# barathanaslan/whisper-ipa

Hardware: AMD Instinct MI355X
Metric: audio-seconds/sec transcribed (whisper-small, 30s clips) (higher is better)
Workload: dtype bf16

## Files before the change

### include/wipa.h

```cpp
#ifndef WIPA_H
#define WIPA_H
#include <stddef.h>
#include <stdint.h>
#ifdef __cplusplus
extern "C" {
#endif

typedef void* wipa_stream_t;

enum { WIPA_F32 = 0, WIPA_BF16 = 1, WIPA_FP8_E4M3 = 2  };
enum { WIPA_OK = 0, WIPA_ERR_ARG = -1, WIPA_ERR_HIP = -2, WIPA_ERR_STATE = -3 };

#define WIPA_N_SAMPLES 480000
#define WIPA_N_FRAMES 3000
#define WIPA_N_FFT 400
#define WIPA_HOP 160
#define WIPA_HEAD_DIM 64

int wipa_version(void);
const char* wipa_last_error(void);

int wipa_stream_create(wipa_stream_t* out);
int wipa_stream_create_cu_limited(int n_cus, wipa_stream_t* out);
int wipa_stream_destroy(wipa_stream_t s);
// ... 122 lines not shown
    const float* slabs;
    const float* bias_o;
    const float* ln_w;
    const float* ln_b;
    const void* wq;
    const float* bq;
    const void* kv;
    void* out;
    int64_t slab_stride;
    int32_t n_slabs, B, d, H, Tk, dtype;
    float eps, qk_scale;
    int32_t cross_splits;
} wipa_cross_block_desc;
int wipa_decode_cross_block(const wipa_cross_block_desc* d, wipa_stream_t s);

int wipa_cross_absorbed_splits(int want, int Tk);
int wipa_cross_absorbed_resident_groups_for(int B, int d, int Tk, int n_splits, int64_t budget_bytes);
int wipa_cross_absorbed_resident_groups(int B, int d, int Tk, int n_splits);
size_t wipa_cross_absorbed_scratch_bytes(int B, int d, int Tk);
int wipa_cross_absorbed_init(int d);
int wipa_cross_absorbed_attention(const void* q, int64_t q_row_stride, const void* wkT, const void* xa, const void* wv, const float* bv,
                                  void* out, int64_t out_row_stride, void* scratch, size_t scratch_bytes, int B, int H, int d, int Tk,
                                  float k_scale, int n_splits, wipa_stream_t s);
int wipa_decode_cross_absorbed_block(const wipa_cross_block_desc* c, const void* wkT, const void* wv, const float* bv, void* scratch,
                                     size_t scratch_bytes, wipa_stream_t s);
int wipa_decode_cross_absorbed_block_out(const wipa_cross_block_desc* c, const void* wkT, const void* wv, const float* bv, const void* wo,
                                         const float* bo, float* slabs_out, int64_t slab_stride, void* scratch, size_t scratch_bytes,
                                         wipa_stream_t s);
int wipa_cross_absorbed_stream(const void* xa, void* scratch, size_t scratch_bytes, int B, int H, int d, int Tk, int n_splits,
                               wipa_stream_t s);

int wipa_greedy_step(const float* logits, int64_t ldl, int B, int V, const float* mask_first,
                     const float* mask_always, int32_t* tokens, int64_t ld_tok, const int32_t* pos_dev, int n_init,
                     int eot, float* sum_logprobs, int32_t* not_done, wipa_stream_t s);
int wipa_add_i32(int32_t* p, int32_t v, wipa_stream_t s);
int wipa_greedy_step_embed(const float* logits, int64_t ldl, int B, int V, const float* mask_first, const float* mask_always,
                           int32_t* tokens, int64_t ld_tok, int32_t* pos_dev, int64_t* posd_dev, int32_t* done_counter, int n_init,
                           int eot, float* sum_logprobs, int32_t* not_done, const void* tok_emb, int emb_dtype,
                           const float* emb_scale, const float* pos_emb, int n_ctx, float* x, const float* ln_w, const float* ln_b,
                           void* y, int y_dtype, int D, float eps, wipa_stream_t s);
#define WIPA_GREEDY_PARTS 2048
int wipa_logits_greedy_supported(int B, int V, int d, int dtype);
size_t wipa_logits_greedy_partials_bytes(int B);
int wipa_logits_greedy(const void* x, int64_t ldx, const void* w, int64_t ldw, float* logits, int64_t ldl, int B, int V, int d,
                       const float* mask_first, const float* mask_always, const int32_t* pos_dev, int n_init, float* partials,
                       size_t partials_bytes, wipa_stream_t s);
// ... 105 lines not shown
```

### whisper_ipa_amd/_lib.py

```python
from __future__ import annotations

import ctypes as C
import os
import threading

_HERE = os.path.dirname(os.path.abspath(__file__))
LIB_PATH = os.path.join(_HERE, "libwipa.so")

WIPA_F32, WIPA_BF16, WIPA_FP8_E4M3 = 0, 1, 2
GREEDY_PARTS = 2048
ENC_GLOBAL, ENC_PER_LAYER = 7, 14
DEC_GLOBAL, DEC_PER_LAYER, DEC_FP8_PER_LAYER = 4, 20, 6
GEMM_DISPATCH = ("tile128", "tile256", "tile384", "tile384n", "tile256p", "skinny", "skinny_fp8", "skinny_ln", "kmajor", "split_k",
                 "tile_fp8", "tile_fp8_384")
ENC_FP8_PER_LAYER = 8
DEC_ABSORBED_PER_LAYER = 1

c_void_p, c_int, c_int64, c_size_t, c_float = C.c_void_p, C.c_int, C.c_int64, C.c_size_t, C.c_float


class GemmDesc(C.Structure):
    _fields_ = [
        ("A", c_void_p), ("W", c_void_p), ("C", c_void_p), ("bias", c_void_p), ("residual", c_void_p),
        ("pos", c_void_p), ("c_offset_dev", c_void_p),
# ... 76 lines not shown
                               c_float, c_void_p]),
    "wipa_layernorm_fp8": (c_int, [c_void_p, c_int64, c_void_p, c_int64, c_void_p, c_void_p, c_void_p, c_int, c_int, c_float, c_void_p]),
    "wipa_rowquant_fp8": (c_int, [c_void_p, c_int, c_int64, c_void_p, c_int64, c_void_p, c_int, c_int, c_void_p]),
    "wipa_add_slabs_layernorm": (c_int, [c_void_p, c_int64, c_void_p, c_int, c_int64, c_void_p, c_int, c_int64, c_void_p,
                                         c_void_p, c_int, c_int, c_float, c_void_p]),
    "wipa_embed_tokens": (c_int, [c_void_p, c_int64, c_int, c_int, c_int, c_void_p, c_void_p, c_int, c_void_p, c_void_p, c_void_p,
                                  c_int, c_void_p]),
    "wipa_attention": (c_int, [_P(AttnDesc), c_void_p]),
    "wipa_flash_attn_enc_f32": (c_int, [c_void_p, c_int64, c_void_p, c_int64, c_void_p, c_int64, c_void_p, c_int64, c_int, c_int,
                                       c_int, c_int, c_void_p]),
    "wipa_flash_attn_enc_bf16": (c_int, [c_void_p, c_int64, c_void_p, c_int64, c_void_p, c_int64, c_int, c_int, c_int,
                                         c_void_p]),
    "wipa_decode_attn": (c_int, [_P(AttnDesc), c_void_p]),
    "wipa_decode_cross_attn": (c_int, [c_void_p, c_void_p, c_void_p, c_int, c_int, c_int, c_int, c_void_p]),
    "wipa_decode_self_block": (c_int, [_P(SelfBlockDesc), c_void_p]),
    "wipa_decode_cross_block": (c_int, [_P(CrossBlockDesc), c_void_p]),
    "wipa_cross_absorbed_splits": (c_int, [c_int, c_int]),
    "wipa_cross_absorbed_resident_groups_for": (c_int, [c_int, c_int, c_int, c_int, c_int64]),
    "wipa_cross_absorbed_resident_groups": (c_int, [c_int, c_int, c_int, c_int]),
    "wipa_cross_absorbed_scratch_bytes": (c_size_t, [c_int, c_int, c_int]),
    "wipa_cross_absorbed_init": (c_int, [c_int]),
    "wipa_cross_absorbed_attention": (c_int, [c_void_p, c_int64, c_void_p, c_void_p, c_void_p, c_void_p, c_void_p, c_int64, c_void_p, c_size_t,
                                              c_int, c_int, c_int, c_int, c_float, c_int, c_void_p]),
    "wipa_cross_absorbed_stream": (c_int, [c_void_p, c_void_p, c_size_t, c_int, c_int, c_int, c_int, c_int, c_void_p]),
    "wipa_decode_cross_absorbed_block": (c_int, [_P(CrossBlockDesc), c_void_p, c_void_p, c_void_p, c_void_p, c_size_t, c_void_p]),
    "wipa_decode_cross_absorbed_block_out": (c_int, [_P(CrossBlockDesc), c_void_p, c_void_p, c_void_p, c_void_p, c_void_p, c_void_p, c_int64,
                                                     c_void_p, c_size_t, c_void_p]),
    "wipa_greedy_step": (c_int, [c_void_p, c_int64, c_int, c_int, c_void_p, c_void_p, c_void_p, c_int64, c_void_p, c_int,
                                 c_int, c_void_p, c_void_p, c_void_p]),
    "wipa_add_i32": (c_int, [c_void_p, C.c_int32, c_void_p]),
    "wipa_greedy_step_embed": (c_int, [c_void_p, c_int64, c_int, c_int, c_void_p, c_void_p, c_void_p, c_int64, c_void_p, c_void_p, c_void_p,
                                       c_int, c_int, c_void_p, c_void_p, c_void_p, c_int, c_void_p, c_void_p, c_int, c_void_p, c_void_p,
                                       c_void_p, c_void_p, c_int, c_int, c_float, c_void_p]),
    "wipa_logits_greedy_supported": (c_int, [c_int, c_int, c_int, c_int]),
    "wipa_logits_greedy_partials_bytes": (c_size_t, [c_int]),
    "wipa_logits_greedy": (c_int, [c_void_p, c_int64, c_void_p, c_int64, c_void_p, c_int64, c_int, c_int, c_int, c_void_p, c_void_p, c_void_p,
                                   c_int, c_void_p, c_size_t, c_void_p]),
    "wipa_greedy_step_embed_partials": (c_int, [c_void_p, c_int, c_int, c_void_p, c_int64, c_void_p, c_void_p, c_void_p, c_int, c_int, c_void_p,
                                                c_void_p, c_void_p, c_int, c_void_p, c_void_p, c_int, c_void_p, c_void_p, c_void_p, c_void_p,
                                                c_int, c_int, c_float, c_void_p]),
    "wipa_embed_layernorm": (c_int, [c_void_p, c_int64, c_int, c_void_p, c_void_p, c_int, c_void_p, c_void_p, c_int, c_void_p, c_void_p,
                                     c_void_p, c_void_p, c_int, c_int, c_float, c_void_p]),
    "wipa_bpe_create": (c_void_p, [c_void_p, c_void_p, c_void_p, c_int]),
    "wipa_bpe_free": (None, [c_void_p]),
    "wipa_bpe_encode_piece": (c_int, [c_void_p, C.c_char_p, c_int, c_void_p, c_int]),
    "wipa_bpe_decode": (c_int, [c_void_p, c_void_p, c_int, c_void_p, c_int]),
# ... 68 lines not shown
```

### whisper_ipa_amd/csrc/cross_absorbed.hip

```cpp
#include <cstdlib>
#include <mutex>
#include <type_traits>

#include "attn_stream.h"
#include "wipa_common.h"

namespace {

constexpr int FT = 32;
constexpr long long XA_RESIDENT_MB_SHARED = 16;
constexpr long long XA_RESIDENT_MB_LONE = -1;
typedef __attribute__((address_space(3))) void* lds_ptr_a;
typedef int v2i32 __attribute__((ext_vector_type(2)));

struct AbsParams {
    const __bf16* qp;
    const __bf16* xa;
    float* part_m;
    float* part_l;
    float* part_o;
    int Tk, n_splits, tiles_per_split, H;
    int resident_groups;
};

constexpr int POLICY_DEFAULT = 0, POLICY_NT = 2;

__device__ __forceinline__ int swz(int row) { return (row & 7) << 1; }

template <int D>
struct AbsCfg {
    static constexpr int NW = 4;
    static constexpr int ROWB = D * 2;
    static constexpr int TILE = FT * ROWB;
    static constexpr int SX = NW * 2 * 64 * 4 * (int)sizeof(float);
    static constexpr int NBUF = (3 * TILE + SX <= 160 * 1024) ? 3 : 2;
    static constexpr int SMEM = NBUF * TILE + SX;
};

template <int D>
__global__ __launch_bounds__(512, 1) void cross_absorbed_kernel(AbsParams p) {
    typedef AbsCfg<D> X;
    constexpr int NW = X::NW, ROWB = X::ROWB, TILE = X::TILE, NBUF = X::NBUF;
    constexpr int NDMA = TILE / 1024 / NW;
    constexpr int KS = D / NW / 32;
    constexpr int CT = D / NW / 16;
    static_assert(D % (32 * NW) == 0 && TILE % (1024 * NW) == 0, "width");
    extern __shared__ __attribute__((aligned(1024))) char smem[];
    float* sx = reinterpret_cast<float*>(smem + NBUF * TILE);
    const int tid = threadIdx.x, lane = tid & 63;
    const int wave = __builtin_amdgcn_readfirstlane(tid >> 6);
    const int l15 = lane & 15, g = lane >> 4;
    const int split = blockIdx.x, b = blockIdx.y;
    const int tile0 = split * p.tiles_per_split;
    const int n_tiles_total = (p.Tk + FT - 1) / FT;
    const int nt = max(0, min(p.tiles_per_split, n_tiles_total - tile0));
    const __bf16* xb = p.xa + (int64_t)b * p.Tk * D;

    bf16x8 qf[KS];
    {
        const __bf16* qr = p.qp + ((int64_t)b * 16 + l15) * D + wave * (D / NW) + 8 * g;
#pragma unroll
        for (int ks = 0; ks < KS; ++ks) qf[ks] = *reinterpret_cast<const bf16x8*>(qr + 32 * ks);
    }
    const __amdgpu_buffer_rsrc_t rX = __builtin_amdgcn_make_buffer_rsrc((void*)xb, 0, 0x7fffffff, 0x00020000);
    int drow[NDMA], dch[NDMA];
#pragma unroll
    for (int i = 0; i < NDMA; ++i) {
        const int off = 1024 * (NDMA * wave + i) + 16 * lane;
        drow[i] = off / ROWB;
        dch[i] = ((off % ROWB) >> 4) ^ swz(off / ROWB);
    }
    const int res_tiles = p.resident_groups / 2;
    auto stage_as = [&](auto policy, int t, int buf) {
        constexpr int AUX = decltype(policy)::value;
        const int f0 = (tile0 + t) * FT;
#pragma unroll
        for (int i = 0; i < NDMA; ++i) {
            const int voff = min(f0 + drow[i], p.Tk - 1) * ROWB + dch[i] * 16;
            __builtin_amdgcn_raw_ptr_buffer_load_lds(rX, (lds_ptr_a)(smem + buf * TILE + 1024 * (NDMA * wave + i)), 16, voff, 0, 0, AUX);
// ... 156 lines not shown
typedef __bf16 bf16x4v __attribute__((ext_vector_type(4)));

template <int D, int NW_>
struct AbsCfg2 {
    static constexpr int NWV = NW_;
    static constexpr int GF = 16;
    static constexpr int ROWB = D * 2;
    static constexpr int SLOT = GF * ROWB;
    static constexpr int SMEM_LOOP = NWV * 2 * SLOT;
    static constexpr int MROW = D + 4;
    static constexpr int SMEM_MERGE = NWV * 16 * MROW * 4 + NWV * 32 * 4;
    static constexpr int SMEM = SMEM_LOOP > SMEM_MERGE ? SMEM_LOOP : SMEM_MERGE;
};

#define WIPA_TR8(X, A, IMM)                                                                                                          \
    asm volatile("ds_read_b64_tr_b16 %0, %8 offset:" #IMM "\n\tds_read_b64_tr_b16 %1, %9 offset:" #IMM                              \
                 "\n\tds_read_b64_tr_b16 %2, %10 offset:" #IMM "\n\tds_read_b64_tr_b16 %3, %11 offset:" #IMM                          \
                 "\n\tds_read_b64_tr_b16 %4, %12 offset:" #IMM "\n\tds_read_b64_tr_b16 %5, %13 offset:" #IMM                          \
                 "\n\tds_read_b64_tr_b16 %6, %14 offset:" #IMM "\n\tds_read_b64_tr_b16 %7, %15 offset:" #IMM "\n\ts_waitcnt lgkmcnt(0)" \
                 : "=&v"(X[0]), "=&v"(X[1]), "=&v"(X[2]), "=&v"(X[3]), "=&v"(X[4]), "=&v"(X[5]), "=&v"(X[6]), "=&v"(X[7])           \
                 : "v"(A[0]), "v"(A[1]), "v"(A[2]), "v"(A[3]), "v"(A[4]), "v"(A[5]), "v"(A[6]), "v"(A[7])                           \
                 : "memory")

template <int D, int NW_>
__global__ __launch_bounds__(64 * NW_, 1) void cross_absorbed_v2_kernel(AbsParams p) {
    typedef AbsCfg2<D, NW_> X;
    constexpr int NWV = X::NWV, GF = X::GF, ROWB = X::ROWB, SLOT = X::SLOT;
    constexpr int NDMA = SLOT / 1024;
    constexpr int KS = D / 32;
    constexpr int CT = D / 16;
    static_assert(SLOT % 1024 == 0 && NDMA <= 32 && CT % 8 == 0 && KS % 4 == 0 && CT / 8 <= 8 && D % 128 == 0, "width");
    extern __shared__ __attribute__((aligned(1024))) char smem[];
    const int tid = threadIdx.x, lane = tid & 63;
    const int wave = __builtin_amdgcn_readfirstlane(tid >> 6);
    const int l15 = lane & 15, g = lane >> 4;
    const int split = blockIdx.x, b = blockIdx.y;
    const int groups_total = (p.Tk + GF - 1) / GF;
    const int gps = 2 * p.tiles_per_split;
    const int g0 = split * gps;
    const int ng = max(0, min(gps, groups_total - g0));
    const int my_n = ng > wave ? (ng - wave + NWV - 1) / NWV : 0;
    const __bf16* xb = p.xa + (int64_t)b * p.Tk * D;
    char* my = smem + wave * (2 * SLOT);

    bf16x8 qf[KS];
    {
        const __bf16* qr = p.qp + ((int64_t)b * 16 + l15) * D + 8 * g;
#pragma unroll
        for (int ks = 0; ks < KS; ++ks) qf[ks] = *reinterpret_cast<const bf16x8*>(qr + 32 * ks);
    }
    const __amdgpu_buffer_rsrc_t rX = __builtin_amdgcn_make_buffer_rsrc((void*)xb, 0, 0x7fffffff, 0x00020000);
    constexpr int G1K = (ROWB % 1024 == 0) ? 1024 : ((ROWB % 512 == 0) ? 512 : 256);
    constexpr int PER = ROWB / G1K, QR = 1024 / G1K;
    static_assert(NDMA % PER == 0 && PER <= 3 && (QR == 1 || QR == 2 || QR == 4), "transfer / row period");
    int dma_a[PER], dma_b[PER];
#pragma unroll
    for (int t = 0; t < PER; ++t) {
        const int off = 1024 * t + 16 * lane;
        const int r = off / ROWB, c = (off - r * ROWB) >> 4;
        dma_a[t] = (c ^ (r << 1)) << 4;
        dma_b[t] = r * ROWB;
    }
    int lane_v = lane;
    auto stage_as = [&](auto policy, int i_local, int slot) {
        constexpr int AUX = decltype(policy)::value;
// ... 492 lines not shown
        for (int e = tid; e < (16 - CG) * 64; e += 512) qh[CG + (e >> 6)][e & 63] = (__bf16)0.f;
    }
    __syncthreads();
    {
        const bf16x8 a0 = *reinterpret_cast<const bf16x8*>(&qh[l15][8 * g]);
        const bf16x8 a1 = *reinterpret_cast<const bf16x8*>(&qh[l15][32 + 8 * g]);
#pragma unroll
        for (int i = 0; i < NTW; ++i) {
            const int nt = wave * NTW + i;
            if (nt < NT) {
                f32x4 acc = {0.f, 0.f, 0.f, 0.f};
                acc = __builtin_amdgcn_mfma_f32_16x16x32_bf16(a0, wkf[i][0], acc, 0, 0, 0);
                acc = __builtin_amdgcn_mfma_f32_16x16x32_bf16(a1, wkf[i][1], acc, 0, 0, 0);
#pragma unroll
                for (int r = 0; r < 4; ++r) {
                    const int bb_ = b0 + 4 * g + r;
                    if (4 * g + r < CG && bb_ < p.B) p.qp[((int64_t)bb_ * 16 + h) * D + 16 * nt + l15] = (__bf16)(acc[r] * p.k_scale);
                }
            }
        }
    }
}

template <int D>
int launch_attn(const AbsParams& p_in, int B, hipStream_t s) {
    const char* e = getenv("WIPA_ABS_KERNEL");
    AbsParams p = p_in;
    p.resident_groups = wipa_cross_absorbed_resident_groups(B, D, p.Tk, p.n_splits);
    if ((e && atoi(e) == 1) || (D > 768 && !(e && atoi(e) == 2)))
        hipLaunchKernelGGL((cross_absorbed_kernel<D>), dim3(p.n_splits, B), dim3(64 * AbsCfg<D>::NW), AbsCfg<D>::SMEM, s, p);
    else if constexpr (D > 768)
        hipLaunchKernelGGL((cross_absorbed_v2_kernel<D, 2>), dim3(p.n_splits, B), dim3(128), (AbsCfg2<D, 2>::SMEM), s, p);
    else {
        static const int waves = [] { const char* w = getenv("WIPA_ABS_WAVES"); return w ? atoi(w) : 3; }();
        if (waves == 2) hipLaunchKernelGGL((cross_absorbed_v2_kernel<D, 2>), dim3(p.n_splits, B), dim3(128), (AbsCfg2<D, 2>::SMEM), s, p);
        else hipLaunchKernelGGL((cross_absorbed_v2_kernel<D, 3>), dim3(p.n_splits, B), dim3(192), (AbsCfg2<D, 3>::SMEM), s, p);
    }
    return WIPA_OK;
}

AbsParams abs_params(void* scratch, int B, int d, int Tk, int S, int H, const void* xa) {
    char* sc = (char*)scratch;
    AbsParams p = {};
    p.qp = (const __bf16*)sc; p.xa = (const __bf16*)xa;
    p.part_m = (float*)(sc + (size_t)B * 16 * d * 2);
    p.part_l = p.part_m + (size_t)B * S * 16;
    p.part_o = p.part_l + (size_t)B * S * 16;
    p.Tk = Tk; p.n_splits = S; p.H = H;
    const int tiles = (Tk + FT - 1) / FT;
    p.tiles_per_split = (tiles + S - 1) / S;
    return p;
}

template <typename F>
int for_width(int d, F f) {
    if (d == 384) return f(std::integral_constant<int, 384>());
    if (d == 512) return f(std::integral_constant<int, 512>());
    if (d == 768) return f(std::integral_constant<int, 768>());
    if (d == 1024) return f(std::integral_constant<int, 1024>());
    return WIPA_ERR_ARG;
}

}

extern "C" int wipa_cross_absorbed_splits(int want, int Tk) {
    const int tiles = (Tk + FT - 1) / FT;
    static const int dflt = [] { const char* e = getenv("WIPA_ABS_SPLITS"); const int v = e ? atoi(e) : 4; return (v >= 1 && v <= 4) ? v : 4; }();
    int s = (want >= 1 && want <= 4) ? want : dflt;
    if (s > tiles / 2) s = tiles / 2;
    return s < 1 ? 1 : s;
}

extern "C" int wipa_cross_absorbed_resident_groups_for(int B, int d, int Tk, int n_splits, int64_t budget_bytes) {
    if (B < 1 || d < 1 || Tk < 1) return 0;
    const int S = wipa_cross_absorbed_splits(n_splits, Tk);
    const int tiles = (Tk + FT - 1) / FT;
    const int gps = 2 * ((tiles + S - 1) / S);
    if (budget_bytes < 0 || budget_bytes >= (int64_t)B * Tk * d * 2) return gps;
    const int64_t g = budget_bytes / ((int64_t)B * S * 16 * d * 2);
    return g < gps ? (int)g : gps;
}

extern "C" int wipa_cross_absorbed_resident_groups(int B, int d, int Tk, int n_splits) {
    static const int64_t env_mb = [] { const char* e = getenv("WIPA_XA_RESIDENT_MB"); return e ? (int64_t)atoll(e) : (int64_t)INT64_MIN; }();
    const int S = wipa_cross_absorbed_splits(n_splits, Tk);
    int64_t mb = env_mb;
    if (mb == INT64_MIN) mb = (S <= 2) ? XA_RESIDENT_MB_SHARED : XA_RESIDENT_MB_LONE;
    return wipa_cross_absorbed_resident_groups_for(B, d, Tk, S, mb < 0 ? -1 : mb * 1000000);
}

extern "C" size_t wipa_cross_absorbed_scratch_bytes(int B, int d, int Tk) {
    (void)Tk;
    return (size_t)B * 16 * d * 2 + (size_t)B * 4 * 16 * (2 + (size_t)d) * 4 + 1024;
}

extern "C" int wipa_cross_absorbed_init(int d) {
    static std::mutex mu;
    static bool done[4] = {false, false, false, false};
    const int wi = d == 384 ? 0 : d == 512 ? 1 : d == 768 ? 2 : d == 1024 ? 3 : -1;
    if (wi < 0) return WIPA_ERR_ARG;
    std::lock_guard<std::mutex> lk(mu);
    if (done[wi]) return WIPA_OK;
    hipError_t e = hipSuccess;
    for_width(d, [&](auto width) {
        constexpr int D = decltype(width)::value;
        e = hipFuncSetAttribute(reinterpret_cast<const void*>(&cross_absorbed_kernel<D>), hipFuncAttributeMaxDynamicSharedMemorySize,
                                AbsCfg<D>::SMEM);
        if constexpr (D <= 768) {
            if (e == hipSuccess)
                e = hipFuncSetAttribute(reinterpret_cast<const void*>(&cross_absorbed_v2_kernel<D, 3>),
                                        hipFuncAttributeMaxDynamicSharedMemorySize, AbsCfg2<D, 3>::SMEM);
        }
        if (e == hipSuccess)
            e = hipFuncSetAttribute(reinterpret_cast<const void*>(&cross_absorbed_v2_kernel<D, 2>),
                                    hipFuncAttributeMaxDynamicSharedMemorySize, AbsCfg2<D, 2>::SMEM);
        return WIPA_OK;
    });
    WIPA_CHECK_HIP(e);
    done[wi] = true;
    return WIPA_OK;
}

extern "C" int wipa_cross_absorbed_stream(const void* xa, void* scratch, size_t scratch_bytes, int B, int H, int d, int Tk, int n_splits,
                                          wipa_stream_t stream) {
    WIPA_REQUIRE(xa && scratch && B > 0 && H >= 1 && H <= 16 && d == H * 64 && (d == 384 || d == 512 || d == 768 || d == 1024) && Tk >= 1 &&
                     n_splits >= 0 && n_splits <= 4,
                 "wipa_cross_absorbed_stream: bad arguments");
    WIPA_REQUIRE(scratch_bytes >= wipa_cross_absorbed_scratch_bytes(B, d, Tk), "wipa_cross_absorbed_stream: scratch too small");
    const int rc0 = wipa_cross_absorbed_init(d);
    if (rc0 != WIPA_OK) return rc0;
    const int S = wipa_cross_absorbed_splits(n_splits, Tk);
    const AbsParams p = abs_params(scratch, B, d, Tk, S, H, xa);
    const int rc = for_width(d, [&](auto width) { return launch_attn<decltype(width)::value>(p, B, (hipStream_t)stream); });
    if (rc != WIPA_OK) return rc;
    WIPA_LAUNCH_CHECK();
    return WIPA_OK;
}

extern "C" int wipa_cross_absorbed_attention(const void* q, int64_t q_row_stride, const void* wkT, const void* xa, const void* wv,
                                             const float* bv, void* out, int64_t out_row_stride, void* scratch, size_t scratch_bytes,
                                             int B, int H, int d, int Tk, float k_scale, int n_splits, wipa_stream_t stream) {
    WIPA_REQUIRE(q && wkT && xa && wv && bv && out && scratch, "wipa_cross_absorbed_attention: null pointer");
    WIPA_REQUIRE(n_splits >= 0 && n_splits <= 4, "wipa_cross_absorbed_attention: n_splits %d (0 = default, 1..4)", n_splits);
    WIPA_REQUIRE(B > 0 && B <= 65535 && H >= 1 && H <= 16 && d == H * 64 && (d == 384 || d == 512 || d == 768 || d == 1024) && Tk >= 1,
                 "wipa_cross_absorbed_attention: bf16, <= 16 heads of 64, d in {384, 512, 768, 1024} (got H=%d d=%d)", H, d);
    WIPA_REQUIRE(q_row_stride % 8 == 0 && out_row_stride >= d && ((uintptr_t)q % 16) == 0 && ((uintptr_t)xa % 16) == 0 &&
                     ((uintptr_t)wkT % 16) == 0 && ((uintptr_t)wv % 16) == 0 && ((uintptr_t)scratch % 16) == 0,
                 "wipa_cross_absorbed_attention: operands must be 16-byte aligned");
    WIPA_REQUIRE((int64_t)Tk * d * 2 < ((int64_t)1 << 31), "wipa_cross_absorbed_attention: clip too long for 32-bit tile offsets");
    WIPA_REQUIRE(scratch_bytes >= wipa_cross_absorbed_scratch_bytes(B, d, Tk), "wipa_cross_absorbed_attention: scratch too small");
    hipStream_t s = (hipStream_t)stream;
    {
        const int rc0 = wipa_cross_absorbed_init(d);
        if (rc0 != WIPA_OK) return rc0;
    }
    const int S = wipa_cross_absorbed_splits(n_splits, Tk);
    const AbsParams p = abs_params(scratch, B, d, Tk, S, H, xa);
    const dim3 gq(16, (B + 15) / 16, 4), gm(H, (B + WIPA_MERGE_CL - 1) / WIPA_MERGE_CL);
    const char* st_env = getenv("WIPA_ABS_STAGES");
    const int stages = st_env ? atoi(st_env) : 7;
    const int rc = for_width(d, [&](auto width) {
        constexpr int D = decltype(width)::value;
        int rc = WIPA_OK;
        if (stages & 1)
            hipLaunchKernelGGL((cross_absorb_q_kernel<D>), gq, dim3(64), 0, s, (const __bf16*)q, q_row_stride, (const __bf16*)wkT,
                               const_cast<__bf16*>(p.qp), B, H, k_scale);
        if (stages & 2) rc = launch_attn<D>(p, B, s);
        if (rc == WIPA_OK && (stages & 4))
            hipLaunchKernelGGL((cross_merge_proj_kernel<D>), gm, dim3(64 * MergeCfg<D>::NWM), 0, s, p.part_m, p.part_l, p.part_o, S,
                               (const __bf16*)wv, bv, (__bf16*)out, out_row_stride, B);
        return rc;
    });
    if (rc != WIPA_OK) return rc;
    WIPA_LAUNCH_CHECK();
    return WIPA_OK;
}

static int absorbed_block(const wipa_cross_block_desc* c, const void* wkT, const void* wv, const float* bv, const void* wo, const float* bo,
                          float* slabs_out, int64_t slab_stride, void* scratch, size_t scratch_bytes, wipa_stream_t stream);

extern "C" int wipa_decode_cross_absorbed_block(const wipa_cross_block_desc* c, const void* wkT, const void* wv, const float* bv, void* scratch,
                                                size_t scratch_bytes, wipa_stream_t stream) {
    WIPA_REQUIRE(c && c->out, "wipa_decode_cross_absorbed_block: null pointer");
    return absorbed_block(c, wkT, wv, bv, nullptr, nullptr, nullptr, 0, scratch, scratch_bytes, stream);
}

extern "C" int wipa_decode_cross_absorbed_block_out(const wipa_cross_block_desc* c, const void* wkT, const void* wv, const float* bv,
                                                    const void* wo, const float* bo, float* slabs_out, int64_t slab_stride, void* scratch,
                                                    size_t scratch_bytes, wipa_stream_t stream) {
    WIPA_REQUIRE(c && wo && bo && slabs_out && slab_stride >= (int64_t)c->B * c->d && ((uintptr_t)wo % 16) == 0,
                 "wipa_decode_cross_absorbed_block_out: null pointer / short slab stride");
    return absorbed_block(c, wkT, wv, bv, wo, bo, slabs_out, slab_stride, scratch, scratch_bytes, stream);
}

static int absorbed_block(const wipa_cross_block_desc* c, const void* wkT, const void* wv, const float* bv, const void* wo, const float* bo,
                          float* slabs_out, int64_t slab_stride, void* scratch, size_t scratch_bytes, wipa_stream_t stream) {
    WIPA_REQUIRE(c && c->x_in && c->x_out && c->ln_w && c->ln_b && c->wq && c->bq && c->kv && (c->out || wo) && wkT && wv && bv && scratch,
                 "wipa_decode_cross_absorbed_block: null pointer");
// ... 38 lines not shown
```

### whisper_ipa_amd/csrc/runtime.hip

```cpp
#include <algorithm>
#include <cstdarg>
#include <cstdlib>
#include <cstring>
#include <strings.h>
#include <map>
#include <mutex>
#include <tuple>
#include <vector>

#include "wipa_common.h"

static thread_local char g_err[512] = "";
void wipa_set_error(const char* fmt, ...) {
    va_list ap;
    va_start(ap, fmt);
    vsnprintf(g_err, sizeof(g_err), fmt, ap);
    va_end(ap);
}
extern "C" const char* wipa_last_error(void) { return g_err; }
extern "C" int wipa_version(void) { return 100; }

extern "C" int wipa_stream_create_cu_limited(int n_cus, wipa_stream_t* out) {
    int dev = 0, total = 0;
    WIPA_CHECK_HIP(hipGetDevice(&dev));
// ... 264 lines not shown
    size_t x, x2, ln, q, ao, h, slabs, posd, absorbed, greedy_part, total;
};
inline int k_slices_for(int K, int dtype) {
    const int ksteps = K * (int)wipa_dtype_size(dtype) / 64;
    int s = ksteps / 12;
    return s < 1 ? 1 : (s > MAX_SLABS ? MAX_SLABS : s);
}
int decode_mode(const wipa_model_cfg* cfg, int B);
constexpr int MAX_PROMPT = 4;
DecScratch dec_scratch(const wipa_model_cfg* c, int B) {
    const size_t e = wipa_dtype_size(c->dtype), d = c->n_text_state;
    const size_t R = (size_t)B * MAX_PROMPT;
    DecScratch s;
    size_t o = 0;
    s.x = o;    o += align256(R * d * 4);
    s.x2 = o;   o += align256((size_t)B * d * 4);
    s.ln = o;   o += align256(R * d * e);
    s.q = o;    o += align256(R * d * e);
    s.ao = o;   o += align256(R * d * e);
    s.h = o;    o += align256(R * 4 * d * e);
    s.slabs = o; o += align256(std::max((size_t)MAX_SLABS * R, (size_t)c->n_text_head * B) * d * 4);
    s.posd = o; o += 256;
    s.absorbed = o;
    if (c->dec_cross_absorbed) o += align256(wipa_cross_absorbed_scratch_bytes(B, (int)d, c->n_audio_ctx));
    s.greedy_part = o;
    if (wipa_logits_greedy_supported(B, c->n_vocab, (int)d, c->dtype)) o += align256(wipa_logits_greedy_partials_bytes(B));
    s.total = o;
    return s;
}

wipa_dec_layout dec_layout(const wipa_model_cfg* c, int B) {
    const size_t e = wipa_dtype_size(c->dtype);
    const size_t d = c->n_text_state, H = c->n_text_head;
    wipa_dec_layout L;
    size_t o = 0;
    L.ld_tok = c->n_text_ctx + 8;
    L.tokens = o; o += align256((size_t)B * L.ld_tok * 4);
    L.pos = o; o += 256;
    L.not_done = o; o += 256;
    L.sum_logprobs = o; o += align256((size_t)B * 4);
    L.ld_logits = round_up(c->n_vocab, 8);
    L.logits = o; o += align256((size_t)B * L.ld_logits * 4);
    L.cross_kv = o; o += align256(c->dec_cross_absorbed ? (size_t)B * c->n_audio_ctx * d * e
                                                        : (size_t)c->n_text_layer * B * 2 * H * c->n_audio_ctx * 64 * e);
    L.self_kv = o; o += align256((size_t)c->n_text_layer * 3 * B * c->n_text_ctx * d * e);
    L.scratch = o; o += dec_scratch(c, B).total;
    L.total_bytes = o;
// ... 12 lines not shown
    if (b >= B) return;
    const int first4[4] = {i0, i1, i2, i3};
    for (int t = 0; t < n_init; ++t) tokens[(int64_t)b * ld_tok + t] = (t < 4 || !extra) ? first4[t & 3] : extra[t];
}

bool absorbed_block_fused() {
    const char* e = getenv("WIPA_ABS_FUSED_PROLOGUE");
    return !(e && atoi(e) == 0);
}

bool absorbed_merge_out() {
    const char* e = getenv("WIPA_ABS_MERGE_OUT");
    return e && atoi(e) == 1;
}
bool tail_fused() {
    const char* e = getenv("WIPA_DECODE_TAIL");
    return !(e && atoi(e) == 0);
}
thread_local bool t_lean_logits = false;
bool logits_fused(const wipa_model_cfg* cfg, int B) {
    const char* e = getenv("WIPA_LOGITS_FUSED");
    const bool on = !(e && atoi(e) == 0);
    return on && tail_fused() && cfg->dec_w_dtype == 0 && wipa_logits_greedy_supported(B, cfg->n_vocab, cfg->n_text_state, cfg->dtype);
}
int32_t* done_counter_of(char* st, const wipa_dec_layout& L) { return (int32_t*)(st + L.pos + 64); }

int enqueue_step_head(const wipa_model_cfg* cfg, const void* const* w, char* st, const wipa_dec_layout& L, int B, wipa_stream_t stream) {
    const DecScratch S = dec_scratch(cfg, B);
    char* sc = st + L.scratch;
    const void* const* lw0 = w + WIPA_DEC_GLOBAL;
    return wipa_embed_layernorm((const int32_t*)(st + L.tokens), L.ld_tok, B, (const int32_t*)(st + L.pos), w[0], emb_dtype(cfg), emb_scale(cfg, w),
                                (const float*)w[1], cfg->n_text_ctx, (float*)(sc + S.x), (const float*)lw0[0], (const float*)lw0[1], sc + S.ln,
                                cfg->dtype, cfg->n_text_state, 1e-5f, stream);
}

int enqueue_step(const wipa_model_cfg* cfg, const void* const* w, char* st, const wipa_dec_layout& L, int B, int n_init,
                 int eot, const float* mask_first, const float* mask_always, wipa_stream_t stream) {
    const int dt = cfg->dtype;
    const bool tail = tail_fused();
    const size_t e = wipa_dtype_size(dt);
    const int d = cfg->n_text_state, H = cfg->n_text_head, nctx = cfg->n_text_ctx, Ta = cfg->n_audio_ctx;
    const DecScratch S = dec_scratch(cfg, B);
    char* sc = st + L.scratch;
    float* x = (float*)(sc + S.x);
    float* x_other = (float*)(sc + S.x2);
    const bool absorbed = cfg->dec_cross_absorbed != 0;
// ... 271 lines not shown
        {
            wipa_attn_desc a;
            memset(&a, 0, sizeof(a));
            const size_t slot = (size_t)B * nctx * d * e;
            a.q = skv; a.k = skv + slot; a.v = skv + 2 * slot; a.out = ao;
            a.q_bs = (int64_t)nctx * d; a.q_rs = d; a.q_hs = 64;
            a.k_bs = a.q_bs; a.k_rs = d; a.k_hs = 64;
            a.v_bs = a.q_bs; a.v_rs = d; a.v_hs = 64;
            a.o_bs = (int64_t)P * d; a.o_rs = d; a.o_hs = 64;
            a.B = B; a.H = H; a.Tq = P; a.Tk = P; a.causal = 1; a.dtype = dt;
            RT_CALL(wipa_attention(&a, stream));
        }
        RT_CALL(residual_gemm(ao, d, lw[4], lw[5]));
        RT_CALL(ln_step(lw[6], lw[7]));
        {
            wipa_gemm_desc g;
            memset(&g, 0, sizeof(g));
        g.stream_weights = 1;
            g.col_scale_n = d; g.col_scale = QK_SCALE;
            RT_CALL(gemm(ln, d, lw[8], d, q, d, M, d, d, dt, dt, (const float*)lw[9], 0, nullptr, stream, &g));
        }
        if (cfg->dec_cross_absorbed) {
            const void* wkT = w[WIPA_DEC_GLOBAL + WIPA_DEC_PER_LAYER * cfg->n_text_layer + WIPA_DEC_ABSORBED_PER_LAYER * l];
            for (int t = 0; t < P; ++t)
                RT_CALL(wipa_cross_absorbed_attention((const char*)q + (size_t)t * d * e, (int64_t)P * d, wkT, st + L.cross_kv,
                                                      (const char*)lw[10] + (size_t)d * d * e, (const float*)lw[11] + d,
                                                      (char*)ao + (size_t)t * d * e, (int64_t)P * d, sc + S.absorbed, S.greedy_part - S.absorbed, B,
                                                      H, d, Ta, QK_SCALE, cfg->dec_cross_splits, stream));
        } else {
            RT_CALL(wipa_decode_cross_attn_multi(q, ckv, ao, B, H, Ta, P, dt, stream));
        }
        RT_CALL(residual_gemm(ao, d, lw[12], lw[13]));
        RT_CALL(ln_step(lw[14], lw[15]));
        {
            wipa_gemm_desc g;
            memset(&g, 0, sizeof(g));
            g.stream_weights = 1;
            RT_CALL(gemm(ln, d, lw[16], d, hb, 4 * d, M, 4 * d, d, dt, dt, (const float*)lw[17], 1, nullptr, stream, &g));
        }
        RT_CALL(residual_gemm(hb, 4 * d, lw[18], lw[19]));
    }
    RT_CALL(ln_step(w[2], w[3]));
    float* logits = (float*)(st + L.logits);
    RT_CALL(gemm(ln + (size_t)(P - 1) * d * e, (int64_t)P * d, w[0], d, logits, L.ld_logits, B, cfg->n_vocab, d, dt, WIPA_F32, nullptr, 0,
                 nullptr, stream));
    hipLaunchKernelGGL(set_pos_kernel, dim3(1), dim3(1), 0, (hipStream_t)stream, pos, posd, P - 1, d);
    RT_CALL(wipa_greedy_step(logits, L.ld_logits, B, cfg->n_vocab, mask_first, mask_always, tokens, L.ld_tok, pos, n_init,
                             eot, (float*)(st + L.sum_logprobs), (int32_t*)(st + L.not_done), stream));
    hipLaunchKernelGGL(advance_pos_kernel, dim3(1), dim3(1), 0, (hipStream_t)stream, pos, posd, d);
    WIPA_LAUNCH_CHECK();
    return WIPA_OK;
// ... 197 lines not shown
extern "C" int wipa_decoder_prefill(const wipa_model_cfg* cfg, const void* const* w, void* state, size_t state_bytes, int B,
                                    int n_init, int eot, const float* mask_first, const float* mask_always, int use_graph,
                                    wipa_stream_t stream) {
    RT_CALL(cfg_check(cfg));
    SplitScope split_scope(cfg);
    WIPA_REQUIRE(w && state && mask_first && mask_always && B > 0, "wipa_decoder_prefill: bad arguments");
    WIPA_REQUIRE(n_init >= 1 && n_init <= MAX_PROMPT, "wipa_decoder_prefill: 1..%d prompt tokens (got %d)", MAX_PROMPT, n_init);
    W8Scope w8_scope(cfg, w);
    const wipa_dec_layout L = dec_layout(cfg, B);
    RT_CALL(state_fits("wipa_decoder_prefill", L, state_bytes));
    char* st = (char*)state;
    auto enqueue = [&]() -> int {
        if (n_init == 1) {
            if (step_needs_head(cfg, B)) RT_CALL(enqueue_step_head(cfg, w, st, L, B, stream));
            return enqueue_decode_step(cfg, w, st, L, B, n_init, eot, mask_first, mask_always, stream);
        }
        return enqueue_prefill(cfg, w, st, L, B, n_init, eot, mask_first, mask_always, stream);
    };
    hipStream_t s = (hipStream_t)stream;
    RT_CALL(init_before_capture(cfg));
    WIPA_CHECK_HIP(hipMemsetAsync(done_counter_of(st, L), 0, sizeof(int32_t), s));
    if (!use_graph || s == nullptr || !graphs_allowed()) return enqueue();
    hipGraphExec_t exec = nullptr;
    const GraphKey key(state, (const void*)w, (const void*)mask_first, (const void*)mask_always, B, n_init, eot, cfg->dtype * 2 + t_f32_split + 4 * decode_mode(cfg, B) + 16 * cfg->dec_w_dtype + 64 * cfg->dec_cross_absorbed * (absorbed_block_fused() ? 2 : 1) + 256 * (int)tail_fused() + 512 * (int)absorbed_merge_out() + 1024 * cfg->dec_cross_splits + 8192 * (int)(!use_fused_step(cfg, B) && logits_fused(cfg, B)), cfg->weights_generation, 1);
    {
        std::lock_guard<std::mutex> lk(g_graph_mu);
        auto it = g_graphs.find(key);
        if (it != g_graphs.end()) exec = it->second;
    }
    if (!exec) {
        hipGraph_t graph = nullptr;
        WIPA_CHECK_HIP(hipStreamBeginCapture(s, hipStreamCaptureModeRelaxed));
        const int rc = enqueue();
        const hipError_t ee = hipStreamEndCapture(s, &graph);
        if (rc != WIPA_OK) {
            if (graph) hipGraphDestroy(graph);
            return rc;
        }
        WIPA_CHECK_HIP(ee);
        WIPA_CHECK_HIP(hipGraphInstantiate(&exec, graph, nullptr, nullptr, 0));
        WIPA_CHECK_HIP(hipGraphDestroy(graph));
        std::lock_guard<std::mutex> lk(g_graph_mu);
        g_graphs[key] = exec;
    }
    WIPA_CHECK_HIP(hipGraphLaunch(exec, s));
    return WIPA_OK;
}
// ... 118 lines not shown
```

Measured before the change: 27250.

## Batch prefill absorbed cross-attention over all prompt rows in one launch

Replaces the per-prompt-token loop of absorbed cross-attention calls during decoder prefill with one rows-aware launch that handles every prompt row per clip. Blocks map linearly to (clip, row, split), and by default are grouped so that rows sharing a clip land on the same XCD and reuse that clip's encoder states in cache. This removes several launches per layer and repeated re-reads of the audio states, at the cost of larger scratch and padded idle blocks. Prefill runs only once per clip, so the effect on end-to-end throughput is bounded.

```diff
diff --git a/include/wipa.h b/include/wipa.h
--- a/include/wipa.h
+++ b/include/wipa.h
@@ -168,6 +168,10 @@
 int wipa_cross_absorbed_attention(const void* q, int64_t q_row_stride, const void* wkT, const void* xa, const void* wv, const float* bv,
                                   void* out, int64_t out_row_stride, void* scratch, size_t scratch_bytes, int B, int H, int d, int Tk,
                                   float k_scale, int n_splits, wipa_stream_t s);
+size_t wipa_cross_absorbed_scratch_bytes_rows(int B, int rows_per_clip, int d, int Tk);
+int wipa_cross_absorbed_attention_rows(const void* q, int64_t q_row_stride, const void* wkT, const void* xa, const void* wv,
+                                       const float* bv, void* out, int64_t out_row_stride, void* scratch, size_t scratch_bytes, int B,
+                                       int rows_per_clip, int H, int d, int Tk, float k_scale, int n_splits, wipa_stream_t s);
 int wipa_decode_cross_absorbed_block(const wipa_cross_block_desc* c, const void* wkT, const void* wv, const float* bv, void* scratch,
                                      size_t scratch_bytes, wipa_stream_t s);
 int wipa_decode_cross_absorbed_block_out(const wipa_cross_block_desc* c, const void* wkT, const void* wv, const float* bv, const void* wo,
diff --git a/whisper_ipa_amd/_lib.py b/whisper_ipa_amd/_lib.py
--- a/whisper_ipa_amd/_lib.py
+++ b/whisper_ipa_amd/_lib.py
@@ -122,6 +122,9 @@
     "wipa_cross_absorbed_init": (c_int, [c_int]),
     "wipa_cross_absorbed_attention": (c_int, [c_void_p, c_int64, c_void_p, c_void_p, c_void_p, c_void_p, c_void_p, c_int64, c_void_p, c_size_t,
                                               c_int, c_int, c_int, c_int, c_float, c_int, c_void_p]),
+    "wipa_cross_absorbed_scratch_bytes_rows": (c_size_t, [c_int, c_int, c_int, c_int]),
+    "wipa_cross_absorbed_attention_rows": (c_int, [c_void_p, c_int64, c_void_p, c_void_p, c_void_p, c_void_p, c_void_p, c_int64, c_void_p,
+                                                   c_size_t, c_int, c_int, c_int, c_int, c_int, c_float, c_int, c_void_p]),
     "wipa_cross_absorbed_stream": (c_int, [c_void_p, c_void_p, c_size_t, c_int, c_int, c_int, c_int, c_int, c_void_p]),
     "wipa_decode_cross_absorbed_block": (c_int, [_P(CrossBlockDesc), c_void_p, c_void_p, c_void_p, c_void_p, c_size_t, c_void_p]),
     "wipa_decode_cross_absorbed_block_out": (c_int, [_P(CrossBlockDesc), c_void_p, c_void_p, c_void_p, c_void_p, c_void_p, c_void_p, c_int64,
diff --git a/whisper_ipa_amd/csrc/cross_absorbed.hip b/whisper_ipa_amd/csrc/cross_absorbed.hip
--- a/whisper_ipa_amd/csrc/cross_absorbed.hip
+++ b/whisper_ipa_amd/csrc/cross_absorbed.hip
@@ -1,4 +1,5 @@
 #include <cstdlib>
+#include <cstring>
 #include <mutex>
 #include <type_traits>
 
@@ -21,7 +22,32 @@
     float* part_o;
     int Tk, n_splits, tiles_per_split, H;
     int resident_groups;
+    int rows_per_clip, n_clips, row_map;
 };
+
+constexpr int ROW_MAP_NAIVE = 0, ROW_MAP_XCD = 1;
+template <bool ROWS>
+__device__ __forceinline__ bool abs_block_ids(const AbsParams& p, int& split, int& row, int& clip) {
+    if constexpr (!ROWS) {
+        split = blockIdx.x;
+        row = clip = blockIdx.y;
+        return true;
+    } else {
+        const int lin = blockIdx.x, S = p.n_splits, P = p.rows_per_clip;
+        if (p.row_map == ROW_MAP_NAIVE) {
+            row = lin / S;
+            split = lin - row * S;
+            clip = row / P;
+            return true;
+        }
+        const int chunk = lin / (8 * P), j = lin - chunk * (8 * P);
+        const int unit = 8 * chunk + (j & 7);
+        clip = unit / S;
+        split = unit - clip * S;
+        row = clip * P + (j >> 3);
+        return clip < p.n_clips;
+    }
+}
 
 constexpr int POLICY_DEFAULT = 0, POLICY_NT = 2;
 
@@ -37,7 +63,7 @@
     static constexpr int SMEM = NBUF * TILE + SX;
 };
 
-template <int D>
+template <int D, bool ROWS = false>
 __global__ __launch_bounds__(512, 1) void cross_absorbed_kernel(AbsParams p) {
     typedef AbsCfg<D> X;
     constexpr int NW = X::NW, ROWB = X::ROWB, TILE = X::TILE, NBUF = X::NBUF;
@@ -50,11 +76,12 @@
     const int tid = threadIdx.x, lane = tid & 63;
     const int wave = __builtin_amdgcn_readfirstlane(tid >> 6);
     const int l15 = lane & 15, g = lane >> 4;
-    const int split = blockIdx.x, b = blockIdx.y;
+    int split, b, clip;
+    if (!abs_block_ids<ROWS>(p, split, b, clip)) return;
     const int tile0 = split * p.tiles_per_split;
     const int n_tiles_total = (p.Tk + FT - 1) / FT;
     const int nt = max(0, min(p.tiles_per_split, n_tiles_total - tile0));
-    const __bf16* xb = p.xa + (int64_t)b * p.Tk * D;
+    const __bf16* xb = p.xa + (int64_t)clip * p.Tk * D;
 
     bf16x8 qf[KS];
     {
@@ -257,7 +284,7 @@
                  : "v"(A[0]), "v"(A[1]), "v"(A[2]), "v"(A[3]), "v"(A[4]), "v"(A[5]), "v"(A[6]), "v"(A[7])                           \
                  : "memory")
 
-template <int D, int NW_>
+template <int D, int NW_, bool ROWS = false>
 __global__ __launch_bounds__(64 * NW_, 1) void cross_absorbed_v2_kernel(AbsParams p) {
     typedef AbsCfg2<D, NW_> X;
     constexpr int NWV = X::NWV, GF = X::GF, ROWB = X::ROWB, SLOT = X::SLOT;
@@ -269,13 +296,14 @@
     const int tid = threadIdx.x, lane = tid & 63;
     const int wave = __builtin_amdgcn_readfirstlane(tid >> 6);
     const int l15 = lane & 15, g = lane >> 4;
-    const int split = blockIdx.x, b = blockIdx.y;
+    int split, b, clip;
+    if (!abs_block_ids<ROWS>(p, split, b, clip)) return;
     const int groups_total = (p.Tk + GF - 1) / GF;
     const int gps = 2 * p.tiles_per_split;
     const int g0 = split * gps;
     const int ng = max(0, min(gps, groups_total - g0));
     const int my_n = ng > wave ? (ng - wave + NWV - 1) / NWV : 0;
-    const __bf16* xb = p.xa + (int64_t)b * p.Tk * D;
+    const __bf16* xb = p.xa + (int64_t)clip * p.Tk * D;
     char* my = smem + wave * (2 * SLOT);
 
     bf16x8 qf[KS];
@@ -814,31 +842,46 @@
     }
 }
 
+int abs_row_map() {
+    const char* e = getenv("WIPA_ABS_ROW_MAP");
+    return (e && strcmp(e, "naive") == 0) ? ROW_MAP_NAIVE : ROW_MAP_XCD;
+}
+
 template <int D>
 int launch_attn(const AbsParams& p_in, int B, hipStream_t s) {
     const char* e = getenv("WIPA_ABS_KERNEL");
     AbsParams p = p_in;
     p.resident_groups = wipa_cross_absorbed_resident_groups(B, D, p.Tk, p.n_splits);
+    p.n_clips = B;
+    p.row_map = abs_row_map();
+    const bool rows = p.rows_per_clip > 1;
+    const int units = p.n_splits * B;
+    const dim3 grid = !rows ? dim3(p.n_splits, B)
+                            : dim3(p.row_map == ROW_MAP_NAIVE ? units * p.rows_per_clip : (units + 7) / 8 * 8 * p.rows_per_clip);
+    typedef void (*kern_t)(AbsParams);
+    auto launch = [&](kern_t one, kern_t many, int threads, int smem) { hipLaunchKernelGGL(rows ? many : one, grid, dim3(threads), smem, s, p); };
     if ((e && atoi(e) == 1) || (D > 768 && !(e && atoi(e) == 2)))
-        hipLaunchKernelGGL((cross_absorbed_kernel<D>), dim3(p.n_splits, B), dim3(64 * AbsCfg<D>::NW), AbsCfg<D>::SMEM, s, p);
+        launch(cross_absorbed_kernel<D, false>, cross_absorbed_kernel<D, true>, 64 * AbsCfg<D>::NW, AbsCfg<D>::SMEM);
     else if constexpr (D > 768)
-        hipLaunchKernelGGL((cross_absorbed_v2_kernel<D, 2>), dim3(p.n_splits, B), dim3(128), (AbsCfg2<D, 2>::SMEM), s, p);
+        launch(cross_absorbed_v2_kernel<D, 2, false>, cross_absorbed_v2_kernel<D, 2, true>, 128, AbsCfg2<D, 2>::SMEM);
     else {
         static const int waves = [] { const char* w = getenv("WIPA_ABS_WAVES"); return w ? atoi(w) : 3; }();
-        if (waves == 2) hipLaunchKernelGGL((cross_absorbed_v2_kernel<D, 2>), dim3(p.n_splits, B), dim3(128), (AbsCfg2<D, 2>::SMEM), s, p);
-        else hipLaunchKernelGGL((cross_absorbed_v2_kernel<D, 3>), dim3(p.n_splits, B), dim3(192), (AbsCfg2<D, 3>::SMEM), s, p);
+        if (waves == 2) launch(cross_absorbed_v2_kernel<D, 2, false>, cross_absorbed_v2_kernel<D, 2, true>, 128, AbsCfg2<D, 2>::SMEM);
+        else launch(cross_absorbed_v2_kernel<D, 3, false>, cross_absorbed_v2_kernel<D, 3, true>, 192, AbsCfg2<D, 3>::SMEM);
     }
     return WIPA_OK;
 }
 
-AbsParams abs_params(void* scratch, int B, int d, int Tk, int S, int H, const void* xa) {
+AbsParams abs_params(void* scratch, int B, int d, int Tk, int S, int H, const void* xa, int rows_per_clip = 1) {
     char* sc = (char*)scratch;
+    const size_t R = (size_t)B * rows_per_clip;
     AbsParams p = {};
     p.qp = (const __bf16*)sc; p.xa = (const __bf16*)xa;
-    p.part_m = (float*)(sc + (size_t)B * 16 * d * 2);
-    p.part_l = p.part_m + (size_t)B * S * 16;
-    p.part_o = p.part_l + (size_t)B * S * 16;
+    p.part_m = (float*)(sc + R * 16 * d * 2);
+    p.part_l = p.part_m + R * S * 16;
+    p.part_o = p.part_l + R * S * 16;
     p.Tk = Tk; p.n_splits = S; p.H = H;
+    p.rows_per_clip = rows_per_clip; p.n_clips = B;
     const int tiles = (Tk + FT - 1) / FT;
     p.tiles_per_split = (tiles + S - 1) / S;
     return p;
@@ -881,10 +924,12 @@
     return wipa_cross_absorbed_resident_groups_for(B, d, Tk, S, mb < 0 ? -1 : mb * 1000000);
 }
 
-extern "C" size_t wipa_cross_absorbed_scratch_bytes(int B, int d, int Tk) {
+extern "C" size_t wipa_cross_absorbed_scratch_bytes_rows(int B, int rows_per_clip, int d, int Tk) {
     (void)Tk;
-    return (size_t)B * 16 * d * 2 + (size_t)B * 4 * 16 * (2 + (size_t)d) * 4 + 1024;
-}
+    const size_t R = (size_t)B * rows_per_clip;
+    return R * 16 * d * 2 + R * 4 * 16 * (2 + (size_t)d) * 4 + 1024;
+}
+extern "C" size_t wipa_cross_absorbed_scratch_bytes(int B, int d, int Tk) { return wipa_cross_absorbed_scratch_bytes_rows(B, 1, d, Tk); }
 
 extern "C" int wipa_cross_absorbed_init(int d) {
     static std::mutex mu;
@@ -896,16 +941,17 @@
     hipError_t e = hipSuccess;
     for_width(d, [&](auto width) {
         constexpr int D = decltype(width)::value;
-        e = hipFuncSetAttribute(reinterpret_cast<const void*>(&cross_absorbed_kernel<D>), hipFuncAttributeMaxDynamicSharedMemorySize,
-                                AbsCfg<D>::SMEM);
+        auto raise = [&](auto kernel, int bytes) {
+            if (e == hipSuccess) e = hipFuncSetAttribute(reinterpret_cast<const void*>(kernel), hipFuncAttributeMaxDynamicSharedMemorySize, bytes);
+        };
+        raise(&cross_absorbed_kernel<D, false>, AbsCfg<D>::SMEM);
+        raise(&cross_absorbed_kernel<D, true>, AbsCfg<D>::SMEM);
         if constexpr (D <= 768) {
-            if (e == hipSuccess)
-                e = hipFuncSetAttribute(reinterpret_cast<const void*>(&cross_absorbed_v2_kernel<D, 3>),
-                                        hipFuncAttributeMaxDynamicSharedMemorySize, AbsCfg2<D, 3>::SMEM);
-        }
-        if (e == hipSuccess)
-            e = hipFuncSetAttribute(reinterpret_cast<const void*>(&cross_absorbed_v2_kernel<D, 2>),
-                                    hipFuncAttributeMaxDynamicSharedMemorySize, AbsCfg2<D, 2>::SMEM);
+            raise(&cross_absorbed_v2_kernel<D, 3, false>, AbsCfg2<D, 3>::SMEM);
+            raise(&cross_absorbed_v2_kernel<D, 3, true>, AbsCfg2<D, 3>::SMEM);
+        }
+        raise(&cross_absorbed_v2_kernel<D, 2, false>, AbsCfg2<D, 2>::SMEM);
+        raise(&cross_absorbed_v2_kernel<D, 2, true>, AbsCfg2<D, 2>::SMEM);
         return WIPA_OK;
     });
     WIPA_CHECK_HIP(e);
@@ -929,26 +975,30 @@
     return WIPA_OK;
 }
 
-extern "C" int wipa_cross_absorbed_attention(const void* q, int64_t q_row_stride, const void* wkT, const void* xa, const void* wv,
-                                             const float* bv, void* out, int64_t out_row_stride, void* scratch, size_t scratch_bytes,
-                                             int B, int H, int d, int Tk, float k_scale, int n_splits, wipa_stream_t stream) {
+extern "C" int wipa_cross_absorbed_attention_rows(const void* q, int64_t q_row_stride, const void* wkT, const void* xa, const void* wv,
+                                                  const float* bv, void* out, int64_t out_row_stride, void* scratch, size_t scratch_bytes,
+                                                  int B, int rows_per_clip, int H, int d, int Tk, float k_scale, int n_splits,
+                                                  wipa_stream_t stream) {
     WIPA_REQUIRE(q && wkT && xa && wv && bv && out && scratch, "wipa_cross_absorbed_attention: null pointer");
     WIPA_REQUIRE(n_splits >= 0 && n_splits <= 4, "wipa_cross_absorbed_attention: n_splits %d (0 = default, 1..4)", n_splits);
     WIPA_REQUIRE(B > 0 && B <= 65535 && H >= 1 && H <= 16 && d == H * 64 && (d == 384 || d == 512 || d == 768 || d == 1024) && Tk >= 1,
                  "wipa_cross_absorbed_attention: bf16, <= 16 heads of 64, d in {384, 512, 768, 1024} (got H=%d d=%d)", H, d);
+    WIPA_REQUIRE(rows_per_clip >= 1 && (int64_t)B * rows_per_clip <= 65535,
+                 "wipa_cross_absorbed_attention: rows_per_clip %d: >= 1 and at most 65535 rows in all", rows_per_clip);
     WIPA_REQUIRE(q_row_stride % 8 == 0 && out_row_stride >= d && ((uintptr_t)q % 16) == 0 && ((uintptr_t)xa % 16) == 0 &&
                      ((uintptr_t)wkT % 16) == 0 && ((uintptr_t)wv % 16) == 0 && ((uintptr_t)scratch % 16) == 0,
                  "wipa_cross_absorbed_attention: operands must be 16-byte aligned");
     WIPA_REQUIRE((int64_t)Tk * d * 2 < ((int64_t)1 << 31), "wipa_cross_absorbed_attention: clip too long for 32-bit tile offsets");
-    WIPA_REQUIRE(scratch_bytes >= wipa_cross_absorbed_scratch_bytes(B, d, Tk), "wipa_cross_absorbed_attention: scratch too small");
+    WIPA_REQUIRE(scratch_bytes >= wipa_cross_absorbed_scratch_bytes_rows(B, rows_per_clip, d, Tk), "wipa_cross_absorbed_attention: scratch too small");
     hipStream_t s = (hipStream_t)stream;
     {
         const int rc0 = wipa_cross_absorbed_init(d);
         if (rc0 != WIPA_OK) return rc0;
     }
     const int S = wipa_cross_absorbed_splits(n_splits, Tk);
-    const AbsParams p = abs_params(scratch, B, d, Tk, S, H, xa);
-    const dim3 gq(16, (B + 15) / 16, 4), gm(H, (B + WIPA_MERGE_CL - 1) / WIPA_MERGE_CL);
+    const int R = B * rows_per_clip;
+    const AbsParams p = abs_params(scratch, B, d, Tk, S, H, xa, rows_per_clip);
+    const dim3 gq(16, (R + 15) / 16, 4), gm(H, (R + WIPA_MERGE_CL - 1) / WIPA_MERGE_CL);
     const char* st_env = getenv("WIPA_ABS_STAGES");
     const int stages = st_env ? atoi(st_env) : 7;
     const int rc = for_width(d, [&](auto width) {
@@ -956,16 +1006,23 @@
         int rc = WIPA_OK;
         if (stages & 1)
             hipLaunchKernelGGL((cross_absorb_q_kernel<D>), gq, dim3(64), 0, s, (const __bf16*)q, q_row_stride, (const __bf16*)wkT,
-                               const_cast<__bf16*>(p.qp), B, H, k_scale);
+                               const_cast<__bf16*>(p.qp), R, H, k_scale);
         if (stages & 2) rc = launch_attn<D>(p, B, s);
         if (rc == WIPA_OK && (stages & 4))
             hipLaunchKernelGGL((cross_merge_proj_kernel<D>), gm, dim3(64 * MergeCfg<D>::NWM), 0, s, p.part_m, p.part_l, p.part_o, S,
-                               (const __bf16*)wv, bv, (__bf16*)out, out_row_stride, B);
+                               (const __bf16*)wv, bv, (__bf16*)out, out_row_stride, R);
         return rc;
     });
     if (rc != WIPA_OK) return rc;
     WIPA_LAUNCH_CHECK();
     return WIPA_OK;
+}
+
+extern "C" int wipa_cross_absorbed_attention(const void* q, int64_t q_row_stride, const void* wkT, const void* xa, const void* wv,
+                                             const float* bv, void* out, int64_t out_row_stride, void* scratch, size_t scratch_bytes,
+                                             int B, int H, int d, int Tk, float k_scale, int n_splits, wipa_stream_t stream) {
+    return wipa_cross_absorbed_attention_rows(q, q_row_stride, wkT, xa, wv, bv, out, out_row_stride, scratch, scratch_bytes, B, 1, H, d, Tk,
+                                              k_scale, n_splits, stream);
 }
 
 static int absorbed_block(const wipa_cross_block_desc* c, const void* wkT, const void* wv, const float* bv, const void* wo, const float* bo,
diff --git a/whisper_ipa_amd/csrc/runtime.hip b/whisper_ipa_amd/csrc/runtime.hip
--- a/whisper_ipa_amd/csrc/runtime.hip
+++ b/whisper_ipa_amd/csrc/runtime.hip
@@ -310,7 +310,7 @@
     s.slabs = o; o += align256(std::max((size_t)MAX_SLABS * R, (size_t)c->n_text_head * B) * d * 4);
     s.posd = o; o += 256;
     s.absorbed = o;
-    if (c->dec_cross_absorbed) o += align256(wipa_cross_absorbed_scratch_bytes(B, (int)d, c->n_audio_ctx));
+    if (c->dec_cross_absorbed) o += align256(wipa_cross_absorbed_scratch_bytes_rows(B, MAX_PROMPT, (int)d, c->n_audio_ctx));
     s.greedy_part = o;
     if (wipa_logits_greedy_supported(B, c->n_vocab, (int)d, c->dtype)) o += align256(wipa_logits_greedy_partials_bytes(B));
     s.total = o;
@@ -369,6 +369,12 @@
     const char* e = getenv("WIPA_LOGITS_FUSED");
     const bool on = !(e && atoi(e) == 0);
     return on && tail_fused() && cfg->dec_w_dtype == 0 && wipa_logits_greedy_supported(B, cfg->n_vocab, cfg->n_text_state, cfg->dtype);
+}
+int abs_prefill_variant() {
+    const char* e = getenv("WIPA_ABS_PREFILL");
+    if (e && strcmp(e, "loop") == 0) return 0;
+    const char* m = getenv("WIPA_ABS_ROW_MAP");
+    return (m && strcmp(m, "naive") == 0) ? 2 : 1;
 }
 int32_t* done_counter_of(char* st, const wipa_dec_layout& L) { return (int32_t*)(st + L.pos + 64); }
 
@@ -686,11 +692,17 @@
         }
         if (cfg->dec_cross_absorbed) {
             const void* wkT = w[WIPA_DEC_GLOBAL + WIPA_DEC_PER_LAYER * cfg->n_text_layer + WIPA_DEC_ABSORBED_PER_LAYER * l];
-            for (int t = 0; t < P; ++t)
-                RT_CALL(wipa_cross_absorbed_attention((const char*)q + (size_t)t * d * e, (int64_t)P * d, wkT, st + L.cross_kv,
-                                                      (const char*)lw[10] + (size_t)d * d * e, (const float*)lw[11] + d,
-                                                      (char*)ao + (size_t)t * d * e, (int64_t)P * d, sc + S.absorbed, S.greedy_part - S.absorbed, B,
-                                                      H, d, Ta, QK_SCALE, cfg->dec_cross_splits, stream));
+            if (abs_prefill_variant() != 0) {
+                RT_CALL(wipa_cross_absorbed_attention_rows(q, d, wkT, st + L.cross_kv, (const char*)lw[10] + (size_t)d * d * e,
+                                                           (const float*)lw[11] + d, ao, d, sc + S.absorbed, S.greedy_part - S.absorbed, B, P,
+                                                           H, d, Ta, QK_SCALE, cfg->dec_cross_splits, stream));
+            } else {
+                for (int t = 0; t < P; ++t)
+                    RT_CALL(wipa_cross_absorbed_attention((const char*)q + (size_t)t * d * e, (int64_t)P * d, wkT, st + L.cross_kv,
+                                                          (const char*)lw[10] + (size_t)d * d * e, (const float*)lw[11] + d,
+                                                          (char*)ao + (size_t)t * d * e, (int64_t)P * d, sc + S.absorbed,
+                                                          S.greedy_part - S.absorbed, B, H, d, Ta, QK_SCALE, cfg->dec_cross_splits, stream));
+            }
         } else {
             RT_CALL(wipa_decode_cross_attn_multi(q, ckv, ao, B, H, Ta, P, dt, stream));
         }
@@ -934,7 +946,7 @@
     WIPA_CHECK_HIP(hipMemsetAsync(done_counter_of(st, L), 0, sizeof(int32_t), s));
     if (!use_graph || s == nullptr || !graphs_allowed()) return enqueue();
     hipGraphExec_t exec = nullptr;
-    const GraphKey key(state, (const void*)w, (const void*)mask_first, (const void*)mask_always, B, n_init, eot, cfg->dtype * 2 + t_f32_split + 4 * decode_mode(cfg, B) + 16 * cfg->dec_w_dtype + 64 * cfg->dec_cross_absorbed * (absorbed_block_fused() ? 2 : 1) + 256 * (int)tail_fused() + 512 * (int)absorbed_merge_out() + 1024 * cfg->dec_cross_splits + 8192 * (int)(!use_fused_step(cfg, B) && logits_fused(cfg, B)), cfg->weights_generation, 1);
+    const GraphKey key(state, (const void*)w, (const void*)mask_first, (const void*)mask_always, B, n_init, eot, cfg->dtype * 2 + t_f32_split + 4 * decode_mode(cfg, B) + 16 * cfg->dec_w_dtype + 64 * cfg->dec_cross_absorbed * (absorbed_block_fused() ? 2 : 1) + 256 * (int)tail_fused() + 512 * (int)absorbed_merge_out() + 1024 * cfg->dec_cross_splits + 8192 * (int)(!use_fused_step(cfg, B) && logits_fused(cfg, B)) + 16384 * (cfg->dec_cross_absorbed ? abs_prefill_variant() : 0), cfg->weights_generation, 1);
     {
         std::lock_guard<std::mutex> lk(g_graph_mu);
         auto it = g_graphs.find(key);
```

New measurement: 27150. No clear change (-0.4%).
